# heracles-ec/heracles

Hardware: AMD Instinct MI355X
Metric: map->Cl pairs/sec + mixing-matrix build sec, nside=4096 lmax=6144 (higher is better)
Workload: dtype f64

## Files before the change

heracles_amd/csrc/hx_sht.hip:

```cpp
#include <algorithm>
#include <chrono>
#include <cmath>
#include <cstdlib>

#include <type_traits>

#include "hx_sht_common.h"


namespace hx {
using namespace hxfft;

__global__ void k_init_norm0(int lmax, double2 *__restrict__ coef, double *__restrict__ alpha)
{
    const int t = blockIdx.x * blockDim.x + threadIdx.x;
    const int m = t >> 1, par = t & 1;
    if (m > lmax) return;
    const double dm = m;
    auto a = [dm](double l) { return sqrt((4.0 * l * l - 1.0) / (l * l - dm * dm)); };
    double al = 1.0;
    for (int l = m + par; l <= lmax; l += 2) {
        const double dl = l;
        const double a1 = a(dl + 1.0), a2 = a(dl + 2.0);
        const double A = a1 * a2;
// ... 129 lines not shown
                        } else {
                            fn.x = fn.y = mpN[q]; fs.x = fs.y = mpS[q];
                            if (pw || wsym) { fn.x *= pwN[q]; fs.x *= pwS[q]; fn.y = fn.x; fs.y = fs.x; }
                            z[u][q] = make_double2(fn.x, haveS ? fs.x : 0.0);
                            z[u + 1][q] = make_double2(fn.y, haveS ? fs.y : 0.0);
                        }
                    } else {
                        const int i0 = (j < n ? j : 0) + q * n, i1 = (j + 1 < n ? j + 1 : 0) + q * n;
                        z[u][q] = zp[i0];
                        z[u + 1][q] = zp[i1];
                    }
                }
            }
        };
        auto load_batch = [&](int u0) __attribute__((always_inline)) {
            if (n >= 2) load_batch_t(std::true_type{}, u0);
            else load_batch_t(std::false_type{}, u0);
        };
        auto finish_batch = [&](int u0) __attribute__((always_inline)) {
            if (MODE != 0 || n < 2) return;
#pragma unroll
            for (int u = 0; u < RING_FB; u += 2) {
                const int j = 2 * (tid + ((u0 + u) >> 1) * nt);
                const bool tail = j == n - 1;
                const Pair w = wsy[u >> 1];
#pragma unroll
                for (int q = 0; q < 4; ++q) {
                    const double2 rn = z[u][q], rs = z[u + 1][q];
                    const double nx = wsym ? rn.x * w.x : rn.x, ny = wsym ? rn.y * w.y : rn.y;
                    const double sx = wsym ? rs.x * w.x : rs.x, sy = wsym ? rs.y * w.y : rs.y;
                    z[u][q] = make_double2(tail ? ny : nx, haveS ? (tail ? sy : sx) : 0.0);
                    z[u + 1][q] = make_double2(ny, haveS ? sy : 0.0);
                }
            }
        };
        load_batch(0);
        int4 nd0 = make_int4(0, 0, 0, 0), nd1 = nd0;
        if (nextv) {
            const int4 *dp = reinterpret_cast<const int4 *>(desc + ringn) + (tid >> 30);
            nd0 = dp[0];
            nd1 = dp[1];
        }
        auto lds_barrier = []() __attribute__((always_inline)) {
            __builtin_amdgcn_s_waitcnt(0xc07f);
            __builtin_amdgcn_s_barrier();
        };
        lds_barrier();
        for (int a = tid; a <= (4 * n) >> 6; a += nt) ph_hi[a] = expipi(-(double)(a << 6) / (2.0 * n));
        if (tid < 64) ph_lo[tid] = expipi(-(double)tid / (2.0 * n));
        lds_barrier();
        auto phase = [&](unsigned q) __attribute__((always_inline)) {
            return cmul(ph_hi[q >> 6], ph_lo[q & 63]);
        };
        {
            for (int u0 = 0;;) {
                finish_batch(u0);
#pragma unroll
                for (int u = 0; u < RING_FB; ++u) {
                    const int j = 2 * (tid + ((u0 + u) >> 1) * nt) + (u & 1);
                    const double2 e0 = odd ? csub(z[u][0], z[u][2]) : cadd(z[u][0], z[u][2]);
                    const double2 e1 = odd ? mul_mi(csub(z[u][1], z[u][3])) : cadd(z[u][1], z[u][3]);
                    const double2 t = make_double2(fma(sg, e1.x, e0.x), fma(sg, e1.y, e0.y));
                    const unsigned jc = j < n ? j : 0;
                    const unsigned qn = blu ? mod_by_inv(jc * (unsigned)r + 2u * jc * jc, 4u * (unsigned)n, inv4n) : jc * (unsigned)r;
                    buf[j < n ? lds_slot(j) : MP - 1] = cmul(t, phase(qn));
                }
                u0 += RING_FB;
                if (u0 * nt >= n) break;
                load_batch(u0);
            }
            if (blu)
                for (int j = n + tid; j < M; j += nt) buf[lds_slot(j)] = make_double2(0.0, 0.0);
        }
        __syncthreads();
        if (nextv) {
            auto sc = [](int v) __attribute__((always_inline)) { return __builtin_amdgcn_readfirstlane(v); };
            cur.sN = ((long long)sc(nd0.y) << 32) | (unsigned)sc(nd0.x);
            cur.sS = ((long long)sc(nd0.w) << 32) | (unsigned)sc(nd0.z);
            cur.bhat_off = ((long long)sc(nd1.y) << 32) | (unsigned)sc(nd1.x);
            cur.n = sc(nd1.z);
            cur.rp = sc(nd1.w);
        }
        double2 *out = Y + (long long)c * P.ny + sN + (long long)r * n;
        double *pxN = nullptr, *pxS = nullptr;
        const double *rfN = nullptr, *rfS = nullptr;
        if (MODE == 1 && pixout) {
            pxN = pixout + (long long)c * P.npix + sN + r;
            pxS = pixout + (long long)c * P.npix + (haveS ? sS : sN) + r;
            if (ref) { rfN = ref + (long long)c * P.npix + sN + r; rfS = ref + (long long)c * P.npix + (haveS ? sS : sN) + r; }
        }
        const int kdrop0 = MODE == 0 ? (P.lmax - r) / 4 + 1 : n, kdrop1 = (4 * n - P.lmax - r + 3) / 4;
        auto emit = [&](int k, double2 v) __attribute__((always_inline)) {
            if (MODE == 0 && k >= kdrop0 && k < kdrop1) return;
            if (MODE == 1 && pxN) {
                double fn = v.x, fs = -v.y;
                if (rfN) { fn = rfN[4 * k] - fn; fs = rfS[4 * k] - fs; }
                pxN[4 * k] = fn;
                if (haveS) pxS[4 * k] = fs;
            } else {
                out[k] = v;
            }
        };
        if (!blu) {
            lds_fft_dif(buf, M, twf, P.twN);
            for (int k = tid; k < n; k += nt) emit(k, buf[lds_slot(bitrev(k, p))]);
            continue;
        }
        if (M >= 16) {
            double2 bq[16];
            const int nbf = M >> 4;
#pragma unroll
            for (int j = 0; j < 16; ++j) bq[j] = bh[j * nbf + (tid < nbf ? tid : 0)];
            lds_fft_dif(buf, M, twf, P.twN, tid, nt, true);
#pragma unroll 1
            for (int i = tid; i < nbf; i += nt) {
                double2 x[16];
#pragma unroll
                for (int j = 0; j < 16; ++j) x[j] = buf[lds_slot(16 * i) + j];
                dif_regs<4>(x);
#pragma unroll
                for (int j = 0; j < 16; ++j) {
                    x[j] = cmul(x[j], bq[j]);
                }
                if (i + nt < nbf) {
#pragma unroll
                    for (int j = 0; j < 16; ++j) bq[j] = bh[j * nbf + i + nt];
                }
                dit_inv_regs<4>(x);
#pragma unroll
                for (int j = 0; j < 16; ++j) buf[lds_slot(16 * i) + j] = x[j];
            }
            __syncthreads();
            lds_fft_dit_inv(buf, M, twf, P.twN, tid, nt, true);
        } else {
            lds_fft_dif(buf, M, twf, P.twN, tid, nt);
            for (int j = tid; j < M; j += nt) buf[lds_slot(j)] = cmul(buf[lds_slot(j)], bh[j]);
            __syncthreads();
            lds_fft_dit_inv(buf, M, twf, P.twN, tid, nt);
        }
        for (int k = tid; k < n; k += nt)
            emit(k, cscale(cmul(buf[lds_slot(k)], phase(2u * mod_by_inv((unsigned)k * (unsigned)k, 2u * (unsigned)n, 2.0 * inv4n))), inv));
    }
}

template <int MODE, bool WSYM = false>
__global__ __launch_bounds__(RING_NTMAX) void k_ring_pairfft(PlanDev P, const RingDesc *__restrict__ desc, int nrings, int nb, int M,
                                                             const double *__restrict__ maps, const double *__restrict__ pixw,
                                                             const double2 *__restrict__ zin, double2 *__restrict__ Y,
                                                             double *__restrict__ pixout = nullptr, const double *__restrict__ ref = nullptr)
{
    extern __shared__ double2 buf[];
    __shared__ double2 tw_hi[TW_HI_MAX], tw_lo[64];
    const int MP = lds_fft_slots(M), n = M, p = ilog2(M);
    double2 *ph_hi = buf + 2 * MP, *ph_lo = ph_hi + ring_ph_hi(M);
    const int nt = blockDim.x, nh = nt >> 1;
    const int nitems = ((nrings + 7) >> 3) * nb * 16;
    const TwFactored twf = load_tw_factored(tw_hi, tw_lo, P.tw, P.twN);
    int tid = threadIdx.x;
    for (int a = tid; a <= (4 * n) >> 6; a += nt) ph_hi[a] = expipi(-(double)(a << 6) / (2.0 * n));
    if (tid < 64) ph_lo[tid] = expipi(-(double)tid / (2.0 * n));
    __syncthreads();
    auto phase = [&](unsigned q) __attribute__((always_inline)) { return cmul(ph_hi[q >> 6], ph_lo[q & 63]); };
    auto ring_of = [&](int item) __attribute__((always_inline)) { return ((item >> 4) / nb) * 8 + (item & 7); };
    auto comp_of = [&](int item) __attribute__((always_inline)) { return (item >> 4) % nb; };
    RingDesc cur = RingDesc{0, 0, 0, 1, 0};
    if ((int)blockIdx.x < nitems && ring_of(blockIdx.x) < nrings) cur = desc[ring_of(blockIdx.x)];
    struct __attribute__((aligned(8))) Pair { double x, y; };
    double2 z[RING_FB][4];
    Pair wsy[RING_FB / 2];
    const bool pw = MODE == 0 && !WSYM && pixw != nullptr;
    constexpr bool wsym = MODE == 0 && WSYM;
    auto request = [&](auto U0C, const RingDesc &d, int c) __attribute__((always_inline)) {
        constexpr int U0 = decltype(U0C)::value;
        const bool hS = d.sS >= 0;
        const double *mpN = maps + (long long)c * P.npix + d.sN, *mpS = maps + (long long)c * P.npix + (hS ? d.sS : d.sN);
        const double *pwN = pixw + d.sN, *pwS = pixw + (hS ? d.sS : d.sN);
        const double2 *zp = zin + (long long)c * P.ny + d.sN;
#pragma unroll
        for (int u = U0; u < U0 + RING_FB / 2; u += 2) {
            const int j = 2 * (tid + (u >> 1) * nt), jj = j + 1 < n ? j : 0;
            wsy[u >> 1] = Pair{1.0, 1.0};
            if (MODE == 0 && wsym) wsy[u >> 1] = *reinterpret_cast<const Pair *>(pwN + jj);
#pragma unroll
            for (int q = 0; q < 4; ++q) {
                const int i = jj + q * n;
                if (MODE == 0) {
                    Pair fn = *reinterpret_cast<const Pair *>(mpN + i), fs = *reinterpret_cast<const Pair *>(mpS + i);
                    if (!wsym && pw) {
                        const Pair wn = *reinterpret_cast<const Pair *>(pwN + i), ws = *reinterpret_cast<const Pair *>(pwS + i);
                        fn.x *= wn.x; fn.y *= wn.y; fs.x *= ws.x; fs.y *= ws.y;
                    }
                    z[u][q] = make_double2(fn.x, fn.y);
                    z[u + 1][q] = make_double2(fs.x, fs.y);
                } else {
                    z[u][q] = zp[i];
                    z[u + 1][q] = zp[i + 1];
                }
            }
        }
    };
    auto finish = [&](bool hS) __attribute__((always_inline)) {
        if (MODE != 0) return;
#pragma unroll
        for (int u = 0; u < RING_FB; u += 2) {
            const Pair w = wsy[u >> 1];
#pragma unroll
            for (int q = 0; q < 4; ++q) {
                const double2 rn = z[u][q], rs = z[u + 1][q];
                const double nx = wsym ? rn.x * w.x : rn.x, ny = wsym ? rn.y * w.y : rn.y;
                const double sx = wsym ? rs.x * w.x : rs.x, sy = wsym ? rs.y * w.y : rs.y;
                z[u][q] = make_double2(nx, hS ? sx : 0.0);
                z[u + 1][q] = make_double2(ny, hS ? sy : 0.0);
            }
        }
    };
    using H0 = std::integral_constant<int, 0>;
    using H1 = std::integral_constant<int, RING_FB / 2>;
    bool have_half = false;
    for (int item = blockIdx.x; item < nitems; item += gridDim.x) {
        const int rpair = (item >> 3) & 1;
        const int ring = ring_of(item), c = comp_of(item);
        const int itn = item + gridDim.x, ringn = itn < nitems ? ring_of(itn) : nrings;
        const bool nextv = ringn < nrings;
        if (ring >= nrings) {
            if (nextv) cur = desc[ringn];
            have_half = false;
            continue;
        }
        const long long sN = cur.sN, sS = cur.sS;
        asm volatile("; item" : "+v"(tid));
        const bool haveS = sS >= 0;
        if (!have_half) request(H0{}, cur, c);
        request(H1{}, cur, c);
        int4 nd0 = make_int4(0, 0, 0, 0);
        if (nextv) nd0 = *(reinterpret_cast<const int4 *>(desc + ringn) + (tid >> 30));
        {
        __builtin_amdgcn_s_waitcnt(0xc07f);
        __builtin_amdgcn_s_barrier();
        finish(haveS);
#pragma unroll
        for (int u = 0; u < RING_FB; ++u) {
            const int j = 2 * (tid + (u >> 1) * nt) + (u & 1);
            if (j >= n) continue;
            const double2 e0 = rpair ? csub(z[u][0], z[u][2]) : cadd(z[u][0], z[u][2]);
            const double2 e1 = rpair ? mul_mi(csub(z[u][1], z[u][3])) : cadd(z[u][1], z[u][3]);
            const double2 t0 = cadd(e0, e1);
            buf[lds_slot(j)] = rpair ? cmul(t0, phase((unsigned)j)) : t0;
            buf[MP + lds_slot(j)] = cmul(csub(e0, e1), phase((unsigned)j * (unsigned)(rpair + 2)));
        }
        __syncthreads();
        have_half = false;
        if (nextv) {
            cur.sN = ((long long)__builtin_amdgcn_readfirstlane(nd0.y) << 32) | (unsigned)__builtin_amdgcn_readfirstlane(nd0.x);
            cur.sS = ((long long)__builtin_amdgcn_readfirstlane(nd0.w) << 32) | (unsigned)__builtin_amdgcn_readfirstlane(nd0.z);
            request(H0{}, cur, comp_of(itn));
            have_half = true;
        }
        const int half = tid >= nh ? 1 : 0, gt = tid - half * nh;
        double2 *bh = buf + half * MP;
        lds_fft_dif(bh, M, twf, P.twN, gt, nh);
        const int r = rpair + 2 * half;
        if (MODE == 1 && pixout) {
            double *pxN = pixout + (long long)c * P.npix + sN + r, *pxS = pixout + (long long)c * P.npix + (haveS ? sS : sN) + r;
            if (ref) {
                const double *rfN = ref + (long long)c * P.npix + sN + r, *rfS = ref + (long long)c * P.npix + (haveS ? sS : sN) + r;
                for (int k = gt; k < n; k += nh) {
                    const double2 v = bh[lds_slot(bitrev(k, p))];
                    pxN[4 * k] = rfN[4 * k] - v.x;
                    if (haveS) pxS[4 * k] = rfS[4 * k] + v.y;
                }
            } else {
                for (int k = gt; k < n; k += nh) {
                    const double2 v = bh[lds_slot(bitrev(k, p))];
                    pxN[4 * k] = v.x;
                    if (haveS) pxS[4 * k] = -v.y;
                }
            }
        } else {
            double2 *out = Y + (long long)c * P.ny + sN + (long long)r * n;
            const int kdrop0 = MODE == 0 ? (P.lmax - r) / 4 + 1 : n, kdrop1 = (4 * n - P.lmax - r + 3) / 4;
            for (int k = gt; k < n; k += nh)
                if (k < kdrop0 || k >= kdrop1) *(out + k) = bh[lds_slot(bitrev(k, p))];
        }
        }
    }
}

constexpr int SPLIT_JMAX = 16;

__global__ __launch_bounds__(512) void k_init_bhat_split(PlanDev P, const int *__restrict__ rp_list, int C,
                                                          double2 *__restrict__ bhat)
{
    extern __shared__ double2 buf[];
    const int rp = rp_list[blockIdx.x];
    const int n = P.nsub[rp], M = 2 * C;
    double2 *out = bhat + P.bhat_off[rp];
    auto b_at = [&](int j) {
        const int jj = j < n ? j : (M - j < n ? M - j : -1);
        return jj < 0 ? make_double2(0.0, 0.0) : expipi((double)chirp_num(jj, n) / (double)n);
    };
    for (int half = 0; half < 2; ++half) {
        __syncthreads();
        for (int j = threadIdx.x; j < C; j += blockDim.x) {
            const double2 b0 = b_at(j), b1 = b_at(j + C);
            buf[lds_slot(j)] = half == 0 ? cadd(b0, b1) : cmul(csub(b0, b1), P.tw[j]);
        }
        __syncthreads();
        lds_fft_dif(buf, C, P.tw, P.twN);
        for (int j = threadIdx.x; j < C; j += blockDim.x) out[half * C + j] = buf[lds_slot(j)];
    }
}

template <int MODE>
__global__ __launch_bounds__(512) void k_ring_subdft_split(PlanDev P, const int *__restrict__ rp_list, int C,
                                                            const double *__restrict__ maps, const double *__restrict__ pixw,
                                                            const double2 *__restrict__ zin, double2 *__restrict__ Y,
                                                            double *__restrict__ pixout = nullptr, const double *__restrict__ ref = nullptr)
{
    extern __shared__ double2 buf[];
    const int rp = rp_list[blockIdx.y];
    const int c = blockIdx.z;
    const int n = P.nsub[rp];
    const long long sN = P.startN[rp], sS = P.startS[rp];
    const int M = 2 * C;
    const bool plain = fft_size_for(n) == n;
    const double *mp = maps + (long long)c * P.npix;
    const double2 *zp = zin + (long long)c * P.ny + sN;
    const double2 *bh = P.bhat + (plain ? 0 : P.bhat_off[rp]);
    const double inv = 1.0 / M;
    __shared__ double2 tw_hi[TW_HI_MAX], tw_lo[64];
    const TwFactored twf = load_tw_factored(tw_hi, tw_lo, P.tw, P.twN);
    auto z_at = [&](int j, int q) {
        if (MODE == 0) {
            const long long iN = sN + j + (long long)q * n;
            double fn = mp[iN];
            if (pixw) fn *= pixw[iN];
            double fs = 0.0;
            if (sS >= 0) {
                const long long iS = sS + j + (long long)q * n;
                fs = mp[iS];
                if (pixw) fs *= pixw[iS];
            }
            return make_double2(fn, fs);
        }
        return zp[j + (long long)q * n];
    };
    auto emit = [&](int r, int k, double2 v, bool add) __attribute__((always_inline)) {
        if (MODE == 1 && pixout) {
            const long long iN = (long long)c * P.npix + sN + 4 * k + r, iS = (long long)c * P.npix + sS + 4 * k + r;
            if (add) {
                pixout[iN] += ref ? -v.x : v.x;
                if (sS >= 0) pixout[iS] += ref ? v.y : -v.y;
            } else {
                double fn = v.x, fs = -v.y;
                if (ref) { fn = ref[iN] - fn; if (sS >= 0) fs = ref[iS] - fs; }
                pixout[iN] = fn;
                if (sS >= 0) pixout[iS] = fs;
            }
        } else {
            double2 *o = Y + (long long)c * P.ny + sN + (long long)r * n + k;
            *o = add ? cadd(*o, v) : v;
        }
    };
    auto input = [&](int r, int j) __attribute__((always_inline)) {
        const double2 t = dif4_combine(z_at(j, 0), z_at(j, 1), z_at(j, 2), z_at(j, 3), r);
        const unsigned qn = load_phase_num(j, r, n, !plain);
        return qn ? cmul(t, expipi(-(double)qn / (2.0 * n))) : t;
    };
    for (int r = 0; r < 4; ++r) {
        if (plain) {
            __syncthreads();
#pragma unroll 4
            for (int u = 0; u < SPLIT_JMAX; ++u) {
                const int j = threadIdx.x + u * blockDim.x;
                if (j < n) buf[lds_slot(j)] = input(r, j);
            }
            __syncthreads();
            lds_fft_dif(buf, n, twf, P.twN);
            const int pbits = ilog2(n);
            for (int k = threadIdx.x; k < n; k += blockDim.x) emit(r, k, buf[lds_slot(bitrev(k, pbits))], false);
            continue;
        }
        for (int half = 0; half < 2; ++half) {
            __syncthreads();
#pragma unroll 4
            for (int u = 0; u < SPLIT_JMAX; ++u) {
                const int j = threadIdx.x + u * blockDim.x;
                if (j < C) {
                    double2 v = make_double2(0.0, 0.0);
                    if (j < n) {
                        v = input(r, j);
                        if (half) v = cmul(v, twf[j]);
                    }
                    buf[lds_slot(j)] = v;
                }
            }
            __syncthreads();
            lds_fft_dif(buf, C, twf, P.twN);
            for (int j = threadIdx.x; j < C; j += blockDim.x) buf[lds_slot(j)] = cmul(buf[lds_slot(j)], bh[half * C + j]);
            __syncthreads();
            lds_fft_dit_inv(buf, C, twf, P.twN);
#pragma unroll 4
            for (int u = 0; u < SPLIT_JMAX; ++u) {
                const int k = threadIdx.x + u * blockDim.x;
                if (k < n) {
                    double2 y = buf[lds_slot(k)];
                    if (half) y = cmulc(y, twf[k]);
                    emit(r, k, cscale(cmul(y, expipi(-(double)chirp_num(k, n) / (double)n)), inv), half != 0);
                }
            }
        }
    }
}

__global__ __launch_bounds__(256) void k_synth_spectrum_v(PlanDev P, const double *__restrict__ Fv, int nc, int lmax,
                                                          double2 *__restrict__ Zc, const int *__restrict__ mlim, int rp_hi)
{
    const int rp = blockIdx.x * 4 + (threadIdx.x & 3), rest = threadIdx.x >> 2;
    if (rp >= P.nrp || rp >= rp_hi) return;
    const int c = rest % nc, kk = rest / nc, kstep = (int)(blockDim.x >> 2) / nc;
    if (kk >= kstep) return;
    const int n = P.nsub[rp], nphi = 4 * n;
    const bool shifted = P.shifted[rp] != 0;
    const long long mstride = (long long)P.nrp_pad * 4 * nc;
    const double *row = Fv + (long long)rp * 4 * nc + 4 * c;
    const int mtop = mlim ? min(lmax, mlim[rp]) : lmax;
    for (int k = kk; 2 * k <= nphi; k += kstep) {
        const int k2 = (nphi - k) % nphi;
        double2 an = make_double2(0.0, 0.0), as = an, bn = an, bs = an;
        for (int m = k; m <= mtop; m += nphi) {
            const double2 *b = reinterpret_cast<const double2 *>(row + m * mstride);
            double2 ph = make_double2(1.0, 0.0);
            if (shifted) ph = expipi((double)(m % (2 * nphi)) / (double)nphi);
            const double sc = m == 0 ? 0.5 : 1.0;
            an = cadd(an, cscale(cmul(b[0], ph), sc));
// ... 31 lines not shown
    const long long mstride = (long long)P.nrp_pad * 4 * nc;
    const double *row = Fv + (long long)rp * 4 * nc;
    for (int e = threadIdx.x; e < SPT_M * nc; e += blockDim.x) {
        const int j = e / nc, c = e % nc, m = m0 + j;
        double2 z1 = make_double2(0.0, 0.0), z2 = z1;
        if (m <= mtop) {
            const double2 *b = reinterpret_cast<const double2 *>(row + m * mstride + 4 * c);
            double2 fn = b[0], fs = b[1];
            if (shifted) {
                const double2 ph = expipi((double)(m % (2 * nphi)) / (double)nphi);
                fn = cmul(fn, ph);
                fs = cmul(fs, ph);
            }
            if (m == 0) {
                z1 = cconj(cadd(make_double2(fn.x, 0.0), mul_pi(make_double2(fs.x, 0.0))));
            } else {
                z1 = cconj(cadd(fn, mul_pi(fs)));
                z2 = cconj(cadd(cconj(fn), mul_pi(cconj(fs))));
            }
        }
        spt[c * SPT_M + j] = z1;
        spt[(nc + c) * SPT_M + j] = z2;
    }
    __syncthreads();
    for (int e = threadIdx.x; e < SPT_M * nc; e += blockDim.x) {
        const int c = e / SPT_M, j = e % SPT_M, m = m0 + j;
        double2 *z = Zc + (long long)c * P.ny + P.startN[rp];
        if (2 * m <= nphi) z[m] = spt[c * SPT_M + j];
        if (m > 0 && 2 * m < nphi) z[nphi - m] = spt[(nc + c) * SPT_M + j];
    }
}

}

using namespace hx;

PlanDev hx_plan::dev() const
{
    PlanDev P;
    P.nside = nside; P.lmax = lmax; P.nrp = nrp; P.nrp_pad = nrp_pad; P.twN = twN;
    P.npix = npix; P.ny = ny;
    P.z = z.as<double>(); P.omz = omz.as<double>(); P.sth = sth.as<double>(); P.rwdef = rwdef.as<double>();
    P.nsub = nsub.as<int>(); P.shifted = shifted.as<int>();
    P.startN = startN.as<long long>(); P.startS = startS.as<long long>(); P.bhat_off = bhat_off.as<long long>();
    P.tw = tw.as<double2>(); P.bhat = bhat.as<double2>();
    P.mfac = mfac.as<double>(); P.kfac2 = kfac2.as<double>();
    P.rec0 = nullptr; P.rec2 = nullptr;
    P.wnorm = wnorm; P.hsrc = hsrc; P.hsrc_stride = hsrc_stride; P.hN = eqN;
    P.nssrc = nssrc; P.ns_m0 = ns_m0; P.ns_ms = m_step;
    return P;
}

static int g_lds_fft_cap = 8192;
static int lds_fft_cap() { return g_lds_fft_cap; }
extern "C" int hx_set_max_lds_fft(int points)
{
    if (points < 16 || points > 8192 || (points & (points - 1))) return fail(HX_ERR_ARG, "hx_set_max_lds_fft: a power of two in [16, 8192]");
    g_lds_fft_cap = points;
    return HX_OK;
}

static int plan_tables(hx_plan *pl)
{
    const int lmax = pl->lmax;
    std::vector<double2> tw(std::max(pl->twN / 2, 64));
    for (int k = 0; k < (int)tw.size(); ++k) {
        long double a = -2.0L * 3.141592653589793238462643383279502884L * k / pl->twN;
        tw[k].x = (double)cosl(a); tw[k].y = (double)sinl(a);
    }
    std::vector<double> mfac(lmax + 1), kfac2(lmax + 3, 0.0);
    {
        long double p = 1.0L;
        for (int m = 0; m <= lmax; ++m) {
            if (m > 0) p *= (2.0L * m - 1.0L) / (2.0L * m);
            long double v = sqrtl((2.0L * m + 1.0L) / (4.0L * 3.141592653589793238462643383279502884L) * p);
            mfac[m] = (double)((m & 1) ? -v : v);
        }
        long double k = 1.0L;
        for (int m = 2; m <= lmax + 2; ++m) {
            if (m > 2) k *= sqrtl((2.0L * m) * (2.0L * m - 1.0L) / ((m - 2.0L) * (m + 2.0L))) / 2.0L;
            kfac2[m] = (double)k;
        }
    }
    HX_TRY(upload(pl->tw, tw));
    HX_TRY(upload(pl->mfac, mfac));
    HX_TRY(upload(pl->kfac2, kfac2));
    hipStream_t st = rt().stream;
    HX_TRY(pl->cn0.alloc(sizeof(double2) * (pl->nlm + TABLE_PAD)));
    HX_TRY(pl->al0.alloc(sizeof(double) * (pl->nlm + TABLE_PAD)));
    HX_HIP(hipMemsetAsync(pl->cn0.p, 0, sizeof(double2) * (pl->nlm + TABLE_PAD), st));
    HX_HIP(hipMemsetAsync(pl->al0.p, 0, sizeof(double) * (pl->nlm + TABLE_PAD), st));
    hipLaunchKernelGGL(k_init_norm0, dim3((2 * (lmax + 1) + 63) / 64), dim3(64), 0, st, lmax, pl->cn0.as<double2>(), pl->al0.as<double>());
    (void)hipFuncSetAttribute(reinterpret_cast<const void *>(k_init_bhat), hipFuncAttributeMaxDynamicSharedMemorySize, 160 * 1024);
    (void)hipFuncSetAttribute(reinterpret_cast<const void *>(k_ring_subdft<0, false>), hipFuncAttributeMaxDynamicSharedMemorySize, 156 * 1024);
    (void)hipFuncSetAttribute(reinterpret_cast<const void *>(k_ring_subdft<0, true>), hipFuncAttributeMaxDynamicSharedMemorySize, 156 * 1024);
    (void)hipFuncSetAttribute(reinterpret_cast<const void *>(k_ring_subdft<1, false>), hipFuncAttributeMaxDynamicSharedMemorySize, 156 * 1024);
    (void)hipFuncSetAttribute(reinterpret_cast<const void *>(k_ring_pairfft<0, false>), hipFuncAttributeMaxDynamicSharedMemorySize, 156 * 1024);
    (void)hipFuncSetAttribute(reinterpret_cast<const void *>(k_ring_pairfft<0, true>), hipFuncAttributeMaxDynamicSharedMemorySize, 156 * 1024);
    (void)hipFuncSetAttribute(reinterpret_cast<const void *>(k_ring_pairfft<1, false>), hipFuncAttributeMaxDynamicSharedMemorySize, 156 * 1024);
    (void)hipFuncSetAttribute(reinterpret_cast<const void *>(k_init_bhat_split), hipFuncAttributeMaxDynamicSharedMemorySize, 160 * 1024);
    (void)hipFuncSetAttribute(reinterpret_cast<const void *>(k_ring_subdft_split<0>), hipFuncAttributeMaxDynamicSharedMemorySize, 156 * 1024);
    (void)hipFuncSetAttribute(reinterpret_cast<const void *>(k_ring_subdft_split<1>), hipFuncAttributeMaxDynamicSharedMemorySize, 156 * 1024);
    HX_HIP(hipGetLastError());
    return HX_OK;
}

extern "C" hx_plan *hx_plan_create(int nside, int lmax, int max_comp)
{
    if (ensure_ready() != HX_OK) return nullptr;
    if (nside < 1 || lmax < 0 || max_comp < 1) {
        set_error("hx_plan_create: bad argument");
        return nullptr;
    }
    hx_plan *pl = new hx_plan;
    pl->nside = nside; pl->lmax = lmax; pl->max_comp = max_comp;
    pl->npix = 12LL * nside * nside;
    pl->nrp = 2 * nside;
    pl->nrp_pad = (pl->nrp + 63) / 64 * 64;
    pl->nlm = (long long)(lmax + 1) * (lmax + 2) / 2;
    pl->wnorm = 4.0 * M_PI / (double)pl->npix;
    const long long ns = nside, ncap = 2 * ns * (ns - 1);
    std::vector<double> z(pl->nrp), omz(pl->nrp), sth(pl->nrp), rw(pl->nrp, 1.0);
    std::vector<int> nsub(pl->nrp), shifted(pl->nrp);
    std::vector<long long> sN(pl->nrp), sS(pl->nrp), boff(pl->nrp, -1);
    const double fact2 = 4.0 / (double)pl->npix, fact1 = (double)(2 * ns) * fact2;
    int maxM = 1;
    for (int rp = 0; rp < pl->nrp; ++rp) {
        const int i = rp + 1;
        if (i < nside) {
            double tmp = (double)i * (double)i * fact2;
            z[rp] = 1.0 - tmp; omz[rp] = tmp; sth[rp] = sqrt(tmp * (2.0 - tmp));
            nsub[rp] = i; sN[rp] = 2LL * i * (i - 1); shifted[rp] = 1;
        } else {
            z[rp] = (double)(2 * nside - i) * fact1; omz[rp] = 1.0 - z[rp];
            sth[rp] = sqrt((1.0 - z[rp]) * (1.0 + z[rp]));
            nsub[rp] = nside; sN[rp] = ncap + (long long)(i - nside) * 4 * ns;
            shifted[rp] = ((i - nside) & 1) == 0;
        }
        sS[rp] = i == 2 * nside ? -1 : pl->npix - sN[rp] - 4LL * nsub[rp];
        maxM = std::max(maxM, fft_size_for(nsub[rp]));
    }
    pl->ny = sN[pl->nrp - 1] + 4LL * nsub[pl->nrp - 1];
    const int cap = lds_fft_cap();
    if (maxM > 2 * cap || (maxM > cap && nside > 0 && [&] { for (int rp = 0; rp < pl->nrp; ++rp) if (fft_size_for(nsub[rp]) > cap && fft_size_for(nsub[rp]) == nsub[rp]) return true; return false; }())) {
        set_error("hx_plan_create: nside=%d needs an in-LDS FFT of %d points (limit %d, %d for Bluestein rings); unsupported", nside, maxM, cap, 2 * cap);
        delete pl;
        return nullptr;
    }
    pl->fft_cap = cap;
    {
        std::map<std::pair<int, int>, std::vector<int>> byM;
        for (int rp = pl->nrp - 1; rp >= 0; --rp) {
            const int M = fft_size_for(nsub[rp]);
            const bool pair = M == nsub[rp] && M >= 16 && M <= cap && (2 * (size_t)lds_fft_slots(M) + ring_ph_hi(M) + 64) * sizeof(double2) + 4096 <= 160 * 1024;
            byM[{M, pair ? -1 : 0}].push_back(rp);
        }
        std::vector<int> list;
        for (auto it = byM.rbegin(); it != byM.rend(); ++it) {
            hx_plan::FftClass c;
            c.M = it->first.first; c.big = it->first.second; c.first = (int)list.size(); c.count = (int)it->second.size();
            list.insert(list.end(), it->second.begin(), it->second.end());
            pl->fft_classes.push_back(c);
        }
        if (upload(pl->fft_rp_list, list) != HX_OK) { delete pl; return nullptr; }
        pl->h_fft_rp_list = list;
    }
    pl->twN = std::max(maxM, 2);
    pl->lds_fft = (size_t)lds_fft_slots(std::min(maxM, cap)) * sizeof(double2);
    pl->h_sth = sth; pl->h_z = z; pl->h_nsub = nsub; pl->h_startN = sN; pl->h_startS = sS;
    std::vector<int> blu_list, blu_split;
    long long btot = 0;
    {
        std::map<int, long long> off_of_n;
        for (int rp = 0; rp < pl->nrp; ++rp) {
            int n = nsub[rp], M = fft_size_for(n);
            if (M == n) continue;
            auto it = off_of_n.find(n);
            if (it == off_of_n.end()) {
                it = off_of_n.emplace(n, btot).first;
                btot += M;
                (M > cap ? blu_split : blu_list).push_back(rp);
            }
            boff[rp] = it->second;
        }
    }
    int rc = HX_OK;
    auto chk = [&](int r) { if (rc == HX_OK) rc = r; };
    chk(upload(pl->z, z)); chk(upload(pl->omz, omz)); chk(upload(pl->sth, sth)); chk(upload(pl->rwdef, rw));
    chk(upload(pl->nsub, nsub)); chk(upload(pl->shifted, shifted));
    chk(upload(pl->startN, sN)); chk(upload(pl->startS, sS)); chk(upload(pl->bhat_off, boff));
    {
        std::vector<RingDesc> desc(pl->h_fft_rp_list.size());
        for (size_t k = 0; k < desc.size(); ++k) {
            const int rp = pl->h_fft_rp_list[k];
            desc[k] = RingDesc{sN[rp], sS[rp], boff[rp], nsub[rp], rp};
        }
        chk(upload(pl->fft_desc, desc));
    }
    chk(pl->bhat.alloc(sizeof(double2) * std::max<long long>(btot, 1)));
    if (rc != HX_OK || plan_tables(pl) != HX_OK) { delete pl; return nullptr; }
    hipStream_t st = rt().stream;
    if (!blu_list.empty()) {
        DevBuf d_list;
        if (upload(d_list, blu_list) != HX_OK) { delete pl; return nullptr; }
        hipLaunchKernelGGL(k_init_bhat, dim3((unsigned)blu_list.size()), dim3(512), pl->lds_fft, st, pl->dev(),
                           d_list.as<int>(), pl->bhat.as<double2>());
        (void)hipStreamSynchronize(st);
    }
    if (!blu_split.empty()) {
        DevBuf d_list;
        if (upload(d_list, blu_split) != HX_OK) { delete pl; return nullptr; }
        hipLaunchKernelGGL(k_init_bhat_split, dim3((unsigned)blu_split.size()), dim3(std::min(512, std::max(64, cap / 16))), (size_t)lds_fft_slots(cap) * sizeof(double2), st,
                           pl->dev(), d_list.as<int>(), cap, pl->bhat.as<double2>());
        (void)hipStreamSynchronize(st);
    }
    if (hipStreamSynchronize(st) != hipSuccess || hipGetLastError() != hipSuccess) {
        set_error("hx_plan_create: table initialisation failed");
        delete pl;
        return nullptr;
    }
    return pl;
}

hx_plan *hx::plan_create_equiangular(int N, int lmax)
{
    if (N < 4 || (N & 3) || lmax < 0 || 2 * lmax + 1 >= N) {
        set_error("equiangular plan: N=%d lmax=%d", N, lmax);
        return nullptr;
    }
    hx_plan *pl = new hx_plan;
    pl->nside = 0; pl->lmax = lmax; pl->max_comp = 16;
    pl->npix = 0; pl->ny = 0;
    pl->eqN = N;
    pl->wnorm = 1.0 / N;
    pl->nrp = N / 4;
    pl->nrp_pad = (pl->nrp + 63) / 64 * 64;
    pl->nlm = (long long)(lmax + 1) * (lmax + 2) / 2;
    std::vector<double> z(pl->nrp), omz(pl->nrp), sth(pl->nrp), rw(pl->nrp, 1.0);
    for (int r = 0; r < pl->nrp; ++r) {
        const long double t = 2.0L * 3.141592653589793238462643383279502884L * (r + 0.5L) / N;
        const long double sh = sinl(0.5L * t);
        z[r] = (double)cosl(t); omz[r] = (double)(2.0L * sh * sh); sth[r] = (double)sinl(t);
    }
    pl->h_sth = sth; pl->h_z = z;
    pl->twN = 2;
    int rc = HX_OK;
    auto chk = [&](int r) { if (rc == HX_OK) rc = r; };
    chk(upload(pl->z, z)); chk(upload(pl->omz, omz)); chk(upload(pl->sth, sth)); chk(upload(pl->rwdef, rw));
    if (rc != HX_OK || plan_tables(pl) != HX_OK || hipStreamSynchronize(rt().stream) != hipSuccess) { delete pl; return nullptr; }
    return pl;
}

extern "C" void hx_plan_destroy(hx_plan *plan)
{
    if (!plan) return;
    if (rt().ready) (void)hipStreamSynchronize(rt().stream);
    for (int i = 0; i < hx_plan::NSTAGE; ++i) {
        if (plan->stage_done[i]) (void)hipEventDestroy(plan->stage_done[i]);
    }
    for (int i = 0; i < hx_plan::NUNIT_EV; ++i)
        if (plan->unit_up[i]) (void)hipEventDestroy(plan->unit_up[i]);
    delete plan;
}

extern "C" int hx_plan_release_scratch(hx_plan *pl)
{
    if (!pl) return fail(HX_ERR_ARG, "hx_plan_release_scratch: null plan");
    if (rt().ready) {
        HX_HIP(hipStreamSynchronize(rt().stream));
        if (rt().copy) HX_HIP(hipStreamSynchronize(rt().copy));
    }
    for (int i = 0; i < hx_plan::NSTAGE; ++i) pl->stage[i].release();
    pl->resid_maps.release();
    pl->Y.release();
    pl->F.release();
    pl->partial.release();
    pl->syn_tab.release();
    return HX_OK;
}

extern "C" int64_t hx_plan_scratch_bytes(const hx_plan *pl)
{
    if (!pl) return 0;
    return (int64_t)(pl->stage[0].bytes + pl->stage[1].bytes + pl->stage[2].bytes + pl->resid_maps.bytes + pl->Y.bytes + pl->F.bytes + pl->partial.bytes + pl->rec0.bytes + pl->rec2.bytes + pl->cn0.bytes + pl->al0.bytes + pl->cn2.bytes + pl->al2.bytes +
                     pl->bhat.bytes + pl->syn_tab.bytes);
}

extern "C" int hx_plan_last_chunks(const hx_plan *pl) { return pl ? pl->last_chunks : 0; }

namespace hx {
int ensure_rec2(hx_plan *pl)
{
    if (pl->cn2.p) return HX_OK;
    HX_TRY(pl->cn2.alloc(sizeof(double2) * (pl->nlm + TABLE_PAD)));
    HX_TRY(pl->al2.alloc(sizeof(double) * (pl->nlm + TABLE_PAD)));
    HX_HIP(hipMemsetAsync(pl->cn2.p, 0, sizeof(double2) * (pl->nlm + TABLE_PAD), rt().stream));
    HX_HIP(hipMemsetAsync(pl->al2.p, 0, sizeof(double) * (pl->nlm + TABLE_PAD), rt().stream));
    hipLaunchKernelGGL(k_init_norm2, dim3((pl->lmax + 64) / 64), dim3(64), 0, rt().stream, pl->lmax, pl->cn2.as<double2>(), pl->al2.as<double>());
    HX_HIP(hipGetLastError());
    return HX_OK;
}

template <int MODE>
static int launch_subdft_classes(hx_plan *pl, int nb, const double *d_maps, const double *d_pw, const double2 *zin, double2 *Y, int rp_lo = 0,
                                 int rp_hi = 0x7fffffff, double *pixout = nullptr, const double *ref = nullptr)
{
    for (const auto &cls : pl->fft_classes) {
        hx_plan::FftClass c = cls;
        if (rp_lo > 0 || rp_hi < pl->nrp) {
            const int *b = pl->h_fft_rp_list.data() + cls.first, *e = b + cls.count;
            const int *x = std::lower_bound(b, e, rp_hi, [](int rp, int lim) { return rp >= lim; });
            const int *y = std::lower_bound(b, e, rp_lo, [](int rp, int lim) { return rp >= lim; });
            c.first = cls.first + (int)(x - b);
            c.count = (int)(y - x);
            if (c.count <= 0) continue;
        }
        if (c.big < 0) {
            const int threads = 2 * std::max(64, c.M / 16);
            const size_t lds = (size_t)(2 * lds_fft_slots(c.M) + ring_ph_hi(c.M) + 64) * sizeof(double2);
            const int per_cu = (int)std::max<size_t>(1, std::min<size_t>(512 / threads, (160 * 1024) / (lds + 3 * 1024 + 256)));
            const long long items = ((long long)c.count + 7) / 8 * nb * 16;
            const unsigned groups = (unsigned)std::min<long long>(items, (long long)rt().cus * per_cu);
            if (MODE == 0 && d_pw && pl->pw_mode == 2) {
                hipLaunchKernelGGL((k_ring_pairfft<MODE, MODE == 0>), dim3(groups), dim3(threads), lds, rt().stream,
                                   pl->dev(), pl->fft_desc.as<RingDesc>() + c.first, c.count, nb, c.M, d_maps, d_pw, zin, Y, pixout, ref);
            } else {
                hipLaunchKernelGGL((k_ring_pairfft<MODE, false>), dim3(groups), dim3(threads), lds, rt().stream,
                                   pl->dev(), pl->fft_desc.as<RingDesc>() + c.first, c.count, nb, c.M, d_maps, d_pw, zin, Y, pixout, ref);
            }
            continue;
        }
        if (c.M > pl->fft_cap || c.big) {
            const int C = std::min(c.M, pl->fft_cap), threads = std::min(512, std::max(64, C / SPLIT_JMAX));
            hipLaunchKernelGGL(k_ring_subdft_split<MODE>, dim3(1, c.count, nb), dim3(threads), (size_t)lds_fft_slots(C) * sizeof(double2), rt().stream,
                               pl->dev(), pl->fft_rp_list.as<int>() + c.first, C, d_maps, d_pw, zin, Y, pixout, ref);
            continue;
        }
        const int threads = std::min(RING_NTMAX, std::max(64, c.M / 16));
        const size_t lds = (size_t)(lds_fft_slots(c.M) + ring_ph_hi(c.M) + 64) * sizeof(double2);
        const int per_cu = (int)std::max<size_t>(1, std::min<size_t>(512 / threads, (160 * 1024) / (lds + 3 * 1024 + 256)));
        const long long items = ((long long)c.count + 7) / 8 * nb * 32;
        const unsigned groups = (unsigned)std::min<long long>(items, (long long)rt().cus * per_cu);
        if (MODE == 0 && d_pw && pl->pw_mode == 2) {
            hipLaunchKernelGGL((k_ring_subdft<MODE, MODE == 0>), dim3(groups), dim3(threads), lds, rt().stream,
                               pl->dev(), pl->fft_desc.as<RingDesc>() + c.first, c.count, nb, c.M, d_maps, d_pw, zin, Y, pixout, ref);
        } else {
            hipLaunchKernelGGL((k_ring_subdft<MODE, false>), dim3(groups), dim3(threads), lds, rt().stream,
                               pl->dev(), pl->fft_desc.as<RingDesc>() + c.first, c.count, nb, c.M, d_maps, d_pw, zin, Y, pixout, ref);
        }
    }
    HX_HIP(hipGetLastError());
    return HX_OK;
}

__global__ __launch_bounds__(256) void k_pixw_symmetry(PlanDev P, const double *__restrict__ pixw, int *__restrict__ flag)
{
    const int rp = blockIdx.x, n = P.nsub[rp];
    const long long sN = P.startN[rp], sS = P.startS[rp];
    bool ok = true;
    for (int j = threadIdx.x; j < n; j += blockDim.x) {
        const double w = pixw[sN + j];
#pragma unroll
        for (int q = 1; q < 4; ++q) ok = ok && pixw[sN + j + (long long)q * n] == w;
        if (sS >= 0) {
#pragma unroll
            for (int q = 0; q < 4; ++q) ok = ok && pixw[sS + j + (long long)q * n] == w;
        }
    }
    if (!ok) *flag = 0;
}

int launch_ring_subdft_maps(hx_plan *pl, int nb, const double *d_maps, const double *d_pw, double2 *Y, int rp_lo, int rp_hi)
{
    ProfScope ps("ring_fft");
    if (d_pw && pl->pw_checked != d_pw) HX_TRY(classify_pixel_weights(pl, d_pw));
    return launch_subdft_classes<0>(pl, nb, d_maps, d_pw, nullptr, Y, rp_lo, rp_hi);
}

int classify_pixel_weights(hx_plan *pl, const double *d_pw)
{
    pl->pw_checked = d_pw;
    pl->pw_mode = 0;
    if (!d_pw || pl->nside < 1) return HX_OK;
    HX_TRY(pl->pw_sym.alloc(sizeof(int)));
    HX_HIP(hipMemsetAsync(pl->pw_sym.p, 1, sizeof(int), rt().stream));
    hipLaunchKernelGGL(k_pixw_symmetry, dim3(pl->nrp), dim3(256), 0, rt().stream, pl->dev(), d_pw, pl->pw_sym.as<int>());
    int flag = 0;
    HX_HIP(hipMemcpyAsync(&flag, pl->pw_sym.p, sizeof(int), hipMemcpyDeviceToHost, rt().stream));
    HX_HIP(hipStreamSynchronize(rt().stream));
    pl->pw_mode = flag != 0 ? 2 : 1;
    return HX_OK;
}
}

static int synthesis_batch_valu(hx_plan *pl, int spin, int nb, const double2 *d_alms, double *d_maps, const double *d_ref)
{
    hipStream_t st = rt().stream;
    const int cpu = spin ? 2 : 1;
    PlanDev P = pl->dev();
    const int umax = synth_valu_max_units(spin);
    const size_t fv_pad = (sizeof(double) * (size_t)(pl->lmax + 1) * pl->nrp_pad * 4 * cpu * umax + 255) & ~(size_t)255;
    HX_TRY(pl->F.alloc(fv_pad + sizeof(double2) * (size_t)pl->ny * cpu * umax));
    double *fsyn = pl->F.as<double>();
    double2 *zc = reinterpret_cast<double2 *>(reinterpret_cast<char *>(pl->F.p) + fv_pad);
    for (int c0 = 0; c0 < nb;) {
        int units = umax;
        while (units * cpu > nb - c0) units >>= 1;
        const int nc = units * cpu;
        hx_plan::TaskSet *ts = nullptr;
        HX_TRY(valu_tasks(pl, spin, &ts, synth_valu_task_blocks(spin, units)));
        HX_TRY(launch_synth_valu(pl, spin, units, *ts, d_alms + (size_t)c0 * pl->nlm, fsyn));
        ProfScope ps("ring_fft");
        hipLaunchKernelGGL(k_synth_spectrum_v, dim3((pl->nrp + 3) / 4), dim3(256), 0, st, P, fsyn, nc, pl->lmax, zc, (const int *)nullptr, pl->nrp);
        HX_TRY(launch_subdft_classes<1>(pl, nc, nullptr, nullptr, zc, nullptr, 0, 0x7fffffff, d_maps + (size_t)c0 * pl->npix,
                                        d_ref ? d_ref + (size_t)c0 * pl->npix : nullptr));
        c0 += nc;
    }
    HX_HIP(hipGetLastError());
    return HX_OK;
}

static int synthesis_batch(hx_plan *pl, int spin, int nb, const double2 *d_alms, double *d_maps,
                           const double *d_ref)
{
    hipStream_t st = rt().stream;
    const int cpu = spin ? 2 : 1;
    PlanDev P = pl->dev();
    const int nunits_all = nb / cpu;
    if (nunits_all >= (spin ? 3 : 5)) {
        const int umax = synth_duo_max_units(spin);
        hx_plan::TaskSet *ts = nullptr;
        HX_TRY(synth_duo_tasks(pl, spin, &ts));
        auto sweep_bytes = [&](int units) {
            const double nc = (double)units * cpu;
            return sizeof(double) * (double)(pl->lmax + 1) * pl->nrp_pad * synth_duo_rowlen(spin, units) + sizeof(double2) * (double)pl->ny * nc +
                   (double)synth_duo_table_bytes(pl, spin, units);
        };
        size_t fr = 0, tot = 0;
        if (hipMemGetInfo(&fr, &tot) != hipSuccess) { (void)hipGetLastError(); fr = 0; }
        double avail = 0.92 * ((double)fr + (double)pl->F.bytes + (double)pl->Y.bytes + (double)pl->syn_tab.bytes);
        if (scratch_budget_bytes() > 0.0) avail = std::min(avail, scratch_budget_bytes());
        for (int u0 = 0; u0 < nunits_all;) {
            int units = std::min(umax, nunits_all - u0);
            if (nunits_all - u0 > umax && nunits_all - u0 < umax + (spin ? 3 : 5)) units = (nunits_all - u0 + 1) / 2;
            while (units > 1 && sweep_bytes(units) > avail) --units;
            if (units < (spin ? 3 : 5) && sweep_bytes(units) > avail) units = 0;
            if (units < (spin ? 3 : 5) && (units == 0 || nunits_all - u0 >= (spin ? 3 : 5))) {
                HX_TRY(synthesis_batch_valu(pl, spin, (nunits_all - u0) * cpu, d_alms + (size_t)u0 * cpu * pl->nlm, d_maps + (size_t)u0 * cpu * pl->npix,
                                            d_ref ? d_ref + (size_t)u0 * cpu * pl->npix : nullptr));
                break;
            }
            const int nc = units * cpu, rowlen = synth_duo_rowlen(spin, units);
            const size_t fv_bytes = sizeof(double) * (size_t)(pl->lmax + 1) * pl->nrp_pad * rowlen;
            const size_t zc_bytes = sizeof(double2) * (size_t)pl->ny * nc;
            const size_t fv_pad = (fv_bytes + 255) & ~(size_t)255;
            HX_TRY(pl->F.alloc(fv_pad + zc_bytes));
            HX_TRY(pl->syn_tab.alloc(synth_duo_table_bytes(pl, spin, units)));
            double *fv = pl->F.as<double>();
            double2 *zc = reinterpret_cast<double2 *>(reinterpret_cast<char *>(pl->F.p) + fv_pad);
            HX_TRY(launch_synth_duo(pl, spin, units, *ts, d_alms + (size_t)u0 * cpu * pl->nlm, pl->syn_tab.as<double>(), fv));
            ProfScope ps("ring_fft");
            {
                const int *ml = (spin ? pl->syn_mlim2 : pl->syn_mlim0).as<int>();
                int rp_t = pl->nrp;
                while (rp_t > 0 && 4 * pl->h_nsub[rp_t - 1] >= 2 * pl->lmax + 2) --rp_t;
                if (rp_t > 0)
                    hipLaunchKernelGGL(k_synth_spectrum_v, dim3((rp_t + 3) / 4), dim3(256), 0, st, P, fv, nc, pl->lmax, zc, ml, rp_t);
                if (rp_t < pl->nrp) {
                    const int nphi_max = 4 * pl->h_nsub[pl->nrp - 1];
                    const dim3 grid(pl->nrp - rp_t, (nphi_max / 2 + SPT_M) / SPT_M);
                    hipLaunchKernelGGL(k_synth_spectrum_t, grid, dim3(256), sizeof(double2) * 2 * nc * SPT_M, st, P, fv, nc, pl->lmax, zc, ml, rp_t);
                }
// ... 338 lines not shown
```

Before: 421.7.

## Streamline ring pair-FFT prologue with phase steps, fused weighting, 32-bit addressing

Replaces the per-element twiddle lookups in the ring pair-FFT fill stage with a per-thread base phase times a small precomputed table of per-unroll step phases held in LDS. It also folds the symmetric pixel-weight multiply and the south-zeroing into the radix-4 prologue, and specializes the prologue on rpair at compile time. Global loads and stores now use 32-bit unsigned offsets, and the output loops hoist the bit-reversed slot base so the inner index math is cheaper. This aims to cut integer and address arithmetic and LDS phase reads in a memory-bound kernel. In exchange it uses slightly more LDS and more code, and the step-phase products may differ from direct lookups by a few ulps.

```diff
diff --git a/heracles_amd/csrc/hx_sht.hip b/heracles_amd/csrc/hx_sht.hip
--- a/heracles_amd/csrc/hx_sht.hip
+++ b/heracles_amd/csrc/hx_sht.hip
@@ -305,13 +305,19 @@
     extern __shared__ double2 buf[];
     __shared__ double2 tw_hi[TW_HI_MAX], tw_lo[64];
     const int MP = lds_fft_slots(M), n = M, p = ilog2(M);
-    double2 *ph_hi = buf + 2 * MP, *ph_lo = ph_hi + ring_ph_hi(M);
+    double2 *ph_hi = buf + 2 * MP, *ph_lo = ph_hi + ring_ph_hi(M), *ph_step = ph_lo + 64;
     const int nt = blockDim.x, nh = nt >> 1;
     const int nitems = ((nrings + 7) >> 3) * nb * 16;
     const TwFactored twf = load_tw_factored(tw_hi, tw_lo, P.tw, P.twN);
     int tid = threadIdx.x;
+    static_assert(RING_FB == 8, "ph_step holds 8 steps per r");
     for (int a = tid; a <= (4 * n) >> 6; a += nt) ph_hi[a] = expipi(-(double)(a << 6) / (2.0 * n));
     if (tid < 64) ph_lo[tid] = expipi(-(double)tid / (2.0 * n));
+    if (tid < 3 * RING_FB) {
+        const int rr = tid / RING_FB + 1, u = tid % RING_FB;
+        const long long d = 2ll * nt * (u >> 1) + (u & 1);
+        ph_step[tid] = expipi(-(double)((d * rr) % (4ll * n)) / (2.0 * n));
+    }
     __syncthreads();
     auto phase = [&](unsigned q) __attribute__((always_inline)) { return cmul(ph_hi[q >> 6], ph_lo[q & 63]); };
     auto ring_of = [&](int item) __attribute__((always_inline)) { return ((item >> 4) / nb) * 8 + (item & 7); };
@@ -323,6 +329,11 @@
     Pair wsy[RING_FB / 2];
     const bool pw = MODE == 0 && !WSYM && pixw != nullptr;
     constexpr bool wsym = MODE == 0 && WSYM;
+    auto at = [](auto *base, unsigned off) __attribute__((always_inline)) {
+        using T = std::remove_pointer_t<decltype(base)>;
+        using B = std::conditional_t<std::is_const<T>::value, const char, char>;
+        return reinterpret_cast<T *>(reinterpret_cast<B *>(base) + (off * (unsigned)sizeof(T)));
+    };
     auto request = [&](auto U0C, const RingDesc &d, int c) __attribute__((always_inline)) {
         constexpr int U0 = decltype(U0C)::value;
         const bool hS = d.sS >= 0;
@@ -331,40 +342,63 @@
         const double2 *zp = zin + (long long)c * P.ny + d.sN;
 #pragma unroll
         for (int u = U0; u < U0 + RING_FB / 2; u += 2) {
-            const int j = 2 * (tid + (u >> 1) * nt), jj = j + 1 < n ? j : 0;
+            const unsigned j = 2u * (tid + (u >> 1) * nt), jj = (int)j + 1 < n ? j : 0u;
             wsy[u >> 1] = Pair{1.0, 1.0};
-            if (MODE == 0 && wsym) wsy[u >> 1] = *reinterpret_cast<const Pair *>(pwN + jj);
+            if (MODE == 0 && wsym) wsy[u >> 1] = *reinterpret_cast<const Pair *>(at(pwN, jj));
 #pragma unroll
             for (int q = 0; q < 4; ++q) {
-                const int i = jj + q * n;
+                const unsigned i = jj + q * n;
                 if (MODE == 0) {
-                    Pair fn = *reinterpret_cast<const Pair *>(mpN + i), fs = *reinterpret_cast<const Pair *>(mpS + i);
+                    Pair fn = *reinterpret_cast<const Pair *>(at(mpN, i)), fs = *reinterpret_cast<const Pair *>(at(mpS, i));
                     if (!wsym && pw) {
-                        const Pair wn = *reinterpret_cast<const Pair *>(pwN + i), ws = *reinterpret_cast<const Pair *>(pwS + i);
+                        const Pair wn = *reinterpret_cast<const Pair *>(at(pwN, i)), ws = *reinterpret_cast<const Pair *>(at(pwS, i));
                         fn.x *= wn.x; fn.y *= wn.y; fs.x *= ws.x; fs.y *= ws.y;
                     }
                     z[u][q] = make_double2(fn.x, fn.y);
                     z[u + 1][q] = make_double2(fs.x, fs.y);
                 } else {
-                    z[u][q] = zp[i];
-                    z[u + 1][q] = zp[i + 1];
+                    z[u][q] = *at(zp, i);
+                    z[u + 1][q] = *at(zp, i + 1);
                 }
             }
         }
     };
-    auto finish = [&](bool hS) __attribute__((always_inline)) {
-        if (MODE != 0) return;
-#pragma unroll
-        for (int u = 0; u < RING_FB; u += 2) {
-            const Pair w = wsy[u >> 1];
+    auto fill = [&](auto RPC, bool hS) __attribute__((always_inline)) {
+        constexpr int RP = decltype(RPC)::value;
+        if (MODE == 0 && !hS) {
+#pragma unroll
+            for (int u = 1; u < RING_FB; u += 2)
+#pragma unroll
+                for (int q = 0; q < 4; ++q) z[u][q] = make_double2(0.0, 0.0);
+        }
+        const unsigned j0 = 2u * tid, qmask = 4u * n - 1u;
+        const double2 sa = RP ? phase(j0 & qmask) : make_double2(1.0, 0.0), sb = phase((j0 * (RP + 2)) & qmask);
+        const double2 *sta = ph_step, *stb = ph_step + (RP + 1) * RING_FB;
+#pragma unroll
+        for (int u = 0; u < RING_FB; ++u) {
+            const int j = 2 * (tid + (u >> 1) * nt) + (u & 1);
+            if (j >= n) continue;
+            double2 v[4];
 #pragma unroll
             for (int q = 0; q < 4; ++q) {
-                const double2 rn = z[u][q], rs = z[u + 1][q];
-                const double nx = wsym ? rn.x * w.x : rn.x, ny = wsym ? rn.y * w.y : rn.y;
-                const double sx = wsym ? rs.x * w.x : rs.x, sy = wsym ? rs.y * w.y : rs.y;
-                z[u][q] = make_double2(nx, hS ? sx : 0.0);
-                z[u + 1][q] = make_double2(ny, hS ? sy : 0.0);
-            }
+                if (MODE == 0) {
+                    const double2 rn = z[u & ~1][q], rs = z[u | 1][q];
+                    v[q] = (u & 1) ? make_double2(rn.y, rs.y) : make_double2(rn.x, rs.x);
+                } else {
+                    v[q] = z[u][q];
+                }
+            }
+            const double2 e0 = RP ? csub(v[0], v[2]) : cadd(v[0], v[2]);
+            const double2 e1 = RP ? mul_mi(csub(v[1], v[3])) : cadd(v[1], v[3]);
+            double2 t0 = cadd(e0, e1), t1 = csub(e0, e1);
+            if (wsym) {
+                const double w = (u & 1) ? wsy[u >> 1].y : wsy[u >> 1].x;
+                t0 = cscale(t0, w);
+                t1 = cscale(t1, w);
+            }
+            const int s = lds_slot(j - (u & 1)) + (u & 1);
+            buf[s] = RP ? cmul(t0, u ? cmul(sa, sta[u]) : sa) : t0;
+            buf[MP + s] = cmul(t1, u ? cmul(sb, stb[u]) : sb);
         }
     };
     using H0 = std::integral_constant<int, 0>;
@@ -390,17 +424,8 @@
         {
         __builtin_amdgcn_s_waitcnt(0xc07f);
         __builtin_amdgcn_s_barrier();
-        finish(haveS);
-#pragma unroll
-        for (int u = 0; u < RING_FB; ++u) {
-            const int j = 2 * (tid + (u >> 1) * nt) + (u & 1);
-            if (j >= n) continue;
-            const double2 e0 = rpair ? csub(z[u][0], z[u][2]) : cadd(z[u][0], z[u][2]);
-            const double2 e1 = rpair ? mul_mi(csub(z[u][1], z[u][3])) : cadd(z[u][1], z[u][3]);
-            const double2 t0 = cadd(e0, e1);
-            buf[lds_slot(j)] = rpair ? cmul(t0, phase((unsigned)j)) : t0;
-            buf[MP + lds_slot(j)] = cmul(csub(e0, e1), phase((unsigned)j * (unsigned)(rpair + 2)));
-        }
+        if (rpair) fill(std::integral_constant<int, 1>{}, haveS);
+        else fill(std::integral_constant<int, 0>{}, haveS);
         __syncthreads();
         have_half = false;
         if (nextv) {
@@ -413,27 +438,37 @@
         double2 *bh = buf + half * MP;
         lds_fft_dif(bh, M, twf, P.twN, gt, nh);
         const int r = rpair + 2 * half;
+        const int sgs = lds_slot(bitrev(gt, p));
         if (MODE == 1 && pixout) {
             double *pxN = pixout + (long long)c * P.npix + sN + r, *pxS = pixout + (long long)c * P.npix + (haveS ? sS : sN) + r;
             if (ref) {
                 const double *rfN = ref + (long long)c * P.npix + sN + r, *rfS = ref + (long long)c * P.npix + (haveS ? sS : sN) + r;
-                for (int k = gt; k < n; k += nh) {
-                    const double2 v = bh[lds_slot(bitrev(k, p))];
-                    pxN[4 * k] = rfN[4 * k] - v.x;
-                    if (haveS) pxS[4 * k] = rfS[4 * k] + v.y;
+#pragma unroll 4
+                for (int k0 = 0; k0 < n; k0 += nh) {
+                    const int k = k0 + gt;
+                    if (k >= n) continue;
+                    const double2 v = bh[sgs + lds_slot(bitrev(k0, p))];
+                    *at(pxN, 4u * k) = *at(rfN, 4u * k) - v.x;
+                    if (haveS) *at(pxS, 4u * k) = *at(rfS, 4u * k) + v.y;
                 }
             } else {
-                for (int k = gt; k < n; k += nh) {
-                    const double2 v = bh[lds_slot(bitrev(k, p))];
-                    pxN[4 * k] = v.x;
-                    if (haveS) pxS[4 * k] = -v.y;
+#pragma unroll 4
+                for (int k0 = 0; k0 < n; k0 += nh) {
+                    const int k = k0 + gt;
+                    if (k >= n) continue;
+                    const double2 v = bh[sgs + lds_slot(bitrev(k0, p))];
+                    *at(pxN, 4u * k) = v.x;
+                    if (haveS) *at(pxS, 4u * k) = -v.y;
                 }
             }
         } else {
             double2 *out = Y + (long long)c * P.ny + sN + (long long)r * n;
             const int kdrop0 = MODE == 0 ? (P.lmax - r) / 4 + 1 : n, kdrop1 = (4 * n - P.lmax - r + 3) / 4;
-            for (int k = gt; k < n; k += nh)
-                if (k < kdrop0 || k >= kdrop1) *(out + k) = bh[lds_slot(bitrev(k, p))];
+#pragma unroll 4
+            for (int k0 = 0; k0 < n; k0 += nh) {
+                const int k = k0 + gt;
+                if (k < n && (k < kdrop0 || k >= kdrop1)) *at(out, (unsigned)k) = bh[sgs + lds_slot(bitrev(k0, p))];
+            }
         }
         }
     }
@@ -771,7 +806,7 @@
         std::map<std::pair<int, int>, std::vector<int>> byM;
         for (int rp = pl->nrp - 1; rp >= 0; --rp) {
             const int M = fft_size_for(nsub[rp]);
-            const bool pair = M == nsub[rp] && M >= 16 && M <= cap && (2 * (size_t)lds_fft_slots(M) + ring_ph_hi(M) + 64) * sizeof(double2) + 4096 <= 160 * 1024;
+            const bool pair = M == nsub[rp] && M >= 16 && M <= cap && (2 * (size_t)lds_fft_slots(M) + ring_ph_hi(M) + 64 + 3 * RING_FB) * sizeof(double2) + 4096 <= 160 * 1024;
             byM[{M, pair ? -1 : 0}].push_back(rp);
         }
         std::vector<int> list;
@@ -936,7 +971,7 @@
         }
         if (c.big < 0) {
             const int threads = 2 * std::max(64, c.M / 16);
-            const size_t lds = (size_t)(2 * lds_fft_slots(c.M) + ring_ph_hi(c.M) + 64) * sizeof(double2);
+            const size_t lds = (size_t)(2 * lds_fft_slots(c.M) + ring_ph_hi(c.M) + 64 + 3 * RING_FB) * sizeof(double2);
             const int per_cu = (int)std::max<size_t>(1, std::min<size_t>(512 / threads, (160 * 1024) / (lds + 3 * 1024 + 256)));
             const long long items = ((long long)c.count + 7) / 8 * nb * 16;
             const unsigned groups = (unsigned)std::min<long long>(items, (long long)rt().cus * per_cu);
```

Result: no change. 421.6 (median of 3 runs) (-0.0%).
